# da-moon/noise-erasurecode-plugin

Hardware: AMD Instinct MI355X
Metric: RS(10,4) encode+reconstruct GB/s at 1/8 GPUs; % HBM roofline (higher is better)
Workload: dtype u8

## Files before the change

noise-erasurecode-plugin_amd/csrc/host_pipeline.cpp:

```cpp
#include "host_pipeline.hpp"

#include <algorithm>
#include <atomic>
#include <chrono>
#include <cstdlib>
#include <cstdio>
#include <cstring>
#include <mutex>
#include <new>
#include <string>
#include <utility>
#include <vector>
#if defined(__x86_64__)
#include <emmintrin.h>
#endif

namespace rsmi {

namespace {
constexpr size_t kPart = size_t(1) << 20;
constexpr size_t kPartMin = size_t(1) << 20;
constexpr size_t kChunkBytes = size_t(8) << 20;
size_t round_up(size_t x, size_t a) { return (x + a - 1) / a * a; }

int pool_threads() {
    const char* e = std::getenv("RSMI_COPY_THREADS");
    int t = e ? std::atoi(e) : static_cast<int>(std::thread::hardware_concurrency());
    return std::max(1, std::min(t, 8));
}
}

namespace {
inline void cpu_relax() {
#if defined(__x86_64__) || defined(__i386__)
    __builtin_ia32_pause();
#elif defined(__aarch64__)
    asm volatile("yield");
#endif
}
}

namespace {
bool stage_nt() {
    static const bool on = [] {
        const char* e = std::getenv("RSMI_STAGE_NT");
        return !(e && std::atoi(e) == 0);
    }();
    return on;
}
}

void stage_copy(void* dst, const void* src, size_t n) {
#if defined(__x86_64__)
    if (stage_nt() && n >= 4096) {
        uint8_t* d = static_cast<uint8_t*>(dst);
        const uint8_t* s = static_cast<const uint8_t*>(src);
        const size_t head = (16u - (reinterpret_cast<uintptr_t>(d) & 15u)) & 15u;
        std::memcpy(d, s, head);
        d += head;
        s += head;
        n -= head;
        size_t i = 0;
        for (; i + 64 <= n; i += 64) {
            const __m128i a = _mm_loadu_si128(reinterpret_cast<const __m128i*>(s + i));
            const __m128i b = _mm_loadu_si128(reinterpret_cast<const __m128i*>(s + i + 16));
            const __m128i c = _mm_loadu_si128(reinterpret_cast<const __m128i*>(s + i + 32));
            const __m128i e = _mm_loadu_si128(reinterpret_cast<const __m128i*>(s + i + 48));
            _mm_stream_si128(reinterpret_cast<__m128i*>(d + i), a);
            _mm_stream_si128(reinterpret_cast<__m128i*>(d + i + 16), b);
            _mm_stream_si128(reinterpret_cast<__m128i*>(d + i + 32), c);
            _mm_stream_si128(reinterpret_cast<__m128i*>(d + i + 48), e);
        }
        for (; i + 16 <= n; i += 16)
            _mm_stream_si128(reinterpret_cast<__m128i*>(d + i), _mm_loadu_si128(reinterpret_cast<const __m128i*>(s + i)));
        std::memcpy(d + i, s + i, n - i);
        return;
    }
#endif
    std::memcpy(dst, src, n);
}

namespace {
bool trace_on() {
    static const bool on = [] {
        const char* e = std::getenv("RSMI_TRACE");
        return e && std::atoi(e) != 0;
    }();
    return on;
}
struct TraceCall {
    std::chrono::steady_clock::time_point t[24];
    const char* name[24];
    int n = 0;
};
thread_local TraceCall g_call;
struct TraceTotals {
    std::mutex mu;
    std::vector<std::pair<std::string, std::vector<double>>> phases;
    long calls = 0;
    ~TraceTotals() {
        if (!calls) return;
        std::fprintf(stderr, "RSMI_TRACE %ld calls, median / mean us per phase:\n", calls);
        double total = 0;
        for (auto& p : phases) {
            std::vector<double>& v = p.second;
            double sum = 0;
            for (double x : v) sum += x;
            std::sort(v.begin(), v.end());
            total += v[v.size() / 2];
            std::fprintf(stderr, "  %-28s %8.2f %8.2f  (%zu)\n", p.first.c_str(), v[v.size() / 2], sum / v.size(),
                         v.size());
        }
        std::fprintf(stderr, "  %-28s %8.2f (sum of medians)\n", "total", total);
    }
};
TraceTotals g_totals;
}

void trace_begin() {
    if (!trace_on()) return;
    g_call.n = 0;
    trace_mark("begin");
}

void trace_mark(const char* phase) {
    if (!trace_on() || g_call.n >= 24) return;
    g_call.t[g_call.n] = std::chrono::steady_clock::now();
    g_call.name[g_call.n++] = phase;
}

void trace_end() {
    if (!trace_on() || g_call.n == 0) return;
    trace_mark("end");
    std::lock_guard<std::mutex> lk(g_totals.mu);
    ++g_totals.calls;
    for (int i = 1; i < g_call.n; ++i) {
        const double us = std::chrono::duration<double, std::micro>(g_call.t[i] - g_call.t[i - 1]).count();
        auto it = std::find_if(g_totals.phases.begin(), g_totals.phases.end(),
                               [&](const auto& p) { return p.first == g_call.name[i]; });
        if (it == g_totals.phases.end()) {
            g_totals.phases.push_back({g_call.name[i], {}});
            it = g_totals.phases.end() - 1;
        }
        it->second.push_back(us);
    }
    g_call.n = 0;
}

void stage_fence() {
#if defined(__x86_64__)
    if (stage_nt()) _mm_sfence();
#endif
}

hipError_t wait_event(hipEvent_t ev) {
    static const int spin_us = [] {
        const char* e = std::getenv("RSMI_SYNC_SPIN_US");
        return e ? std::max(0, std::min(std::atoi(e), 100000)) : 200;
    }();
    static const int max_spinners = [] {
        const char* e = std::getenv("RSMI_SYNC_SPINNERS");
        return e ? std::max(0, std::atoi(e)) : 2;
    }();
    static const bool adaptive = [] {
        const char* e = std::getenv("RSMI_SYNC_ADAPTIVE");
        return !(e && std::atoi(e) == 0);
    }();
    static std::atomic<int> spinners{0};
    thread_local bool last_short = true;
    const auto t0 = std::chrono::steady_clock::now();
    if (spin_us > 0 && (last_short || !adaptive)) {
        if (spinners.fetch_add(1, std::memory_order_relaxed) < max_spinners) {
            const auto until = t0 + std::chrono::microseconds(spin_us);
            do {
                const hipError_t q = hipEventQuery(ev);
                if (q != hipErrorNotReady) {
                    spinners.fetch_sub(1, std::memory_order_relaxed);
                    return q;
                }
                cpu_relax();
            } while (std::chrono::steady_clock::now() < until);
        }
        spinners.fetch_sub(1, std::memory_order_relaxed);
    }
    const hipError_t r = hipEventSynchronize(ev);
    last_short = std::chrono::steady_clock::now() - t0 <= std::chrono::microseconds(spin_us);
    return r;
}

namespace {
void copy_pieces(const CopyPool::Piece* b, const CopyPool::Piece* e);
}

struct CopyPool::Async {
    Job job;
    bool queued = false;
};

void CopyPool::split(const std::vector<Piece>& pieces, size_t group_bytes, Job& job) const {
    size_t group = 0;
    job.bounds.push_back(0);
    for (const Piece& p : pieces)
        for (size_t o = 0; o < p.len; o += kPart) {
            const size_t len = std::min(kPart, p.len - o);
            job.pieces.push_back({static_cast<uint8_t*>(p.dst) + o, static_cast<const uint8_t*>(p.src) + o, len, p.nt});
            group += len;
            if (group >= group_bytes) {
                job.bounds.push_back(job.pieces.size());
                group = 0;
// ... 294 lines not shown
```

noise-erasurecode-plugin_amd/csrc/rsmi.cpp:

```cpp
#include "../../include/rsmi.h"

#include <hip/hip_runtime.h>

#include <sched.h>

#include <algorithm>
#include <functional>
#include <atomic>
#include <chrono>
#include <cmath>
#include <cstdio>
#include <thread>
#include <condition_variable>
#include <cstdlib>
#include <cstring>
#include <deque>
#include <map>
#include <memory>
#include <mutex>
#include <new>
#include <shared_mutex>
#include <string>
#include <vector>

// ... 80 lines not shown
    void* p = nullptr;
    size_t cap = 0;
    bool reserve_keep(size_t bytes, size_t used, hipStream_t s) {
        if (bytes <= cap) return true;
        const size_t want = std::max({bytes, size_t(4096), 4 * cap});
        void* np = nullptr;
        if (hipMallocAsync(&np, want, s) != hipSuccess) return false;
        if (p && used &&
            hipMemcpyAsync(np, p, std::min(used, cap), hipMemcpyDeviceToDevice, s) != hipSuccess) {
            (void)hipFreeAsync(np, s);
            return false;
        }
        if (p) (void)hipFreeAsync(p, s);
        p = np;
        cap = want;
        return true;
    }
    bool needs(size_t bytes) const { return bytes > cap; }
    void release() {
        if (p) {
            (void)hipFreeAsync(p, nullptr);
            (void)hipStreamSynchronize(nullptr);
        }
        p = nullptr;
        cap = 0;
    }
};

struct Staging {
    void* p = nullptr;
    void* dev = nullptr;
    size_t cap = 0;
    unsigned flags = hipHostMallocDefault;
    hipEvent_t done = nullptr;
    bool pending = false;
    std::vector<void*> retired;
    bool acquire(size_t bytes) {
        if (pending) {
            (void)hipEventSynchronize(done);
            pending = false;
        }
        if (!done && hipEventCreateWithFlags(&done, hipEventDisableTiming) != hipSuccess) return false;
        if (bytes <= cap) return true;
        const size_t want = std::max({bytes, size_t(1) << 16, 2 * cap});
        void* np = nullptr;
        if (hipHostMalloc(&np, want, flags) != hipSuccess) return false;
        if (p) retired.push_back(p);
        p = np;
        if (hipHostGetDevicePointer(&dev, np, 0) != hipSuccess) dev = np;
        cap = want;
        return true;
    }
    void release_after(hipStream_t s) {
        if (hipEventRecord(done, s) == hipSuccess) pending = true;
    }
    void destroy() {
        if (pending) (void)hipEventSynchronize(done);
        for (void* r : retired) (void)hipHostFree(r);
        retired.clear();
        if (p) (void)hipHostFree(p);
        if (done) (void)hipEventDestroy(done);
        p = nullptr;
        dev = nullptr;
        done = nullptr;
    }
};

}

constexpr size_t kBatchChunks = 4;
constexpr size_t kBatchChunksMax = 8;
constexpr size_t kBatchChunkMin = size_t(16) << 20;

using rsmi::PatKey;

namespace {

struct Lease {
    hipStream_t stream = nullptr;
    hipStream_t stream2 = nullptr;
    hipEvent_t dev_done = nullptr;
    std::atomic<bool> dev_pending{false};
    hipEvent_t ev[kBatchChunksMax] = {};
    Staging st_stripe;
    Staging st_batch, st_pieces;
    Staging st_onepat;
    Staging st_out;
    Staging st_in;
    Staging st_scrub;
    rsmi::MailboxHost* mb = nullptr;
    rsmi::MailboxHost* mb_dev = nullptr;
    rsmi::MailboxDev* mbd = nullptr;
    uint64_t mb_timeout = 0;
    DevBuf d_stripe_pat, d_batch, d_pack, d_pieces, d_onepat, d_scrub;
    std::unique_ptr<rsmi::HostPipeline> pipe;
    std::vector<uint32_t> pid, start;
    std::vector<uint64_t> sort_a, sort_b;
    std::vector<PatKey> miss_keys;
    size_t seen_uploaded = 0;
    uint64_t seen_tables = ~uint64_t(0);

    bool init() {
        static const bool wc = [] {
            const char* e = std::getenv("RSMI_STAGE_WC");
            return e && std::atoi(e) != 0;
        }();
        if (wc) st_in.flags = hipHostMallocWriteCombined;
        if (hipStreamCreateWithFlags(&stream, hipStreamNonBlocking) != hipSuccess) return false;
        if (hipEventCreateWithFlags(&dev_done, hipEventDisableTiming) != hipSuccess) return false;
        for (hipEvent_t& e : ev)
            if (hipEventCreateWithFlags(&e, hipEventDisableTiming) != hipSuccess) return false;
        return true;
    }
    void begin(hipStream_t s) {
        if (dev_pending.load()) (void)hipStreamWaitEvent(s, dev_done, 0);
    }
    void end(hipStream_t s) {
        if (hipEventRecord(dev_done, s) == hipSuccess) dev_pending.store(true);
    }
    rsmi::HostPipeline* pipeline() {
        if (!pipe) pipe.reset(new (std::nothrow) rsmi::HostPipeline());
        return pipe.get();
    }
    hipStream_t chunk_stream(int ch) {
        static const bool two = [] {
            const char* e = std::getenv("RSMI_CHUNK_STREAMS");
            return e && std::atoi(e) == 2;
        }();
        if (!two || ch % 2 == 0) return stream;
        if (!stream2 && hipStreamCreateWithFlags(&stream2, hipStreamNonBlocking) != hipSuccess) stream2 = nullptr;
        return stream2 ? stream2 : stream;
    }
    ~Lease() {
        if (stream2) (void)hipStreamSynchronize(stream2);
        if (stream) (void)hipStreamSynchronize(stream);
        if (dev_pending.load()) (void)hipEventSynchronize(dev_done);
        pipe.reset();
        st_stripe.destroy();
        st_batch.destroy();
        st_pieces.destroy();
        st_onepat.destroy();
        st_out.destroy();
        st_in.destroy();
        st_scrub.destroy();
        for (DevBuf* b : {&d_stripe_pat, &d_batch, &d_pack, &d_pieces, &d_onepat, &d_scrub}) b->release();
        if (mb) (void)hipHostFree(mb);
        if (mbd) (void)hipFree(mbd);
        for (hipEvent_t e : ev)
            if (e) (void)hipEventDestroy(e);
        if (dev_done) (void)hipEventDestroy(dev_done);
        if (stream2) (void)hipStreamDestroy(stream2);
        if (stream) (void)hipStreamDestroy(stream);
    }
};

}

struct rs_ctx {
    int k = 0, n = 0, m = 0, device = 0;
    std::vector<uint8_t> enc;
    rsmi::DeviceSet* set = nullptr;
    bool set_member = false;
    const rsmi::BitsliceKernel* bitslice = nullptr;
    bool bitslice_rec = false;
    int bitslice_rec_min_e = 1;
    uint32_t xcd = 1;
    uint32_t xcd_split_enc = 0;
    uint32_t xcd_split_rec = ~0u;
    std::string rec_name;
    bool inline_desc = true;
    size_t small_split = 16;

    DevBuf d_encpat;
    DevBuf d_gf;

    mutable std::shared_mutex pat_mu;
    rsmi::PatIndex pat_index;
    std::vector<uint32_t> h_cnt;
    std::vector<uint8_t> h_lo;
    std::vector<rsmi::BsStripeMask> h_mask;
    int n_tops = 0;
    std::vector<PatKey> h_key;
    GrowBuf d_pcoef, d_psrc, d_pdst, d_pcnt, d_pstat, d_pkey;
    size_t uploaded = 0;
    size_t pat_cap = 0;
    int test_fail_flush = 0, flush_attempts = 0;
    uint64_t evictions = 0;
    uint64_t tables_gen = 0;
    std::atomic<int64_t> batches_in_place{0}, batches_staged{0};
    std::atomic<int64_t> encodes_in_place{0};
    std::atomic<int64_t> decodes_in_place{0};
    std::atomic<int64_t> rec_stripes_table{0}, rec_stripes_syndrome{0};
    std::atomic<int64_t> encode_batches{0};
    std::atomic<int64_t> mailbox_calls{0}, mailbox_recovered{0};
    std::atomic<int64_t> update_stripes{0}, update_copy_commits{0};
    std::atomic<int64_t> read_regenerated{0}, read_copied{0};
    std::atomic<int64_t> check_stripes{0}, scrub_regenerated{0};
    std::atomic<int64_t> repair_checked{0};
    std::atomic<int64_t> combine_jobs{0}, combine_rows{0};
    std::atomic<int64_t> batch_lens_passes{0};
    std::atomic<int64_t> combine_lens_launches{0};
    std::atomic<int64_t> update_degraded{0}, update_absorbed{0};
    std::atomic<int64_t> column_stripes{0}, column_bytes{0};
    bool repair_fused = true;
    uint32_t xcd_repair = 0;
    uint32_t xcd_update = ~0u;
    hipEvent_t pat_ev = nullptr;
    hipStream_t build_stream = nullptr;
    hipEvent_t caller_ev = nullptr;
    bool build_after_caller = true;
    bool pat_ev_valid = false;
    Staging st_pat;

    std::mutex lease_mu;
    std::condition_variable lease_cv;
    std::vector<std::unique_ptr<Lease>> leases;
    std::deque<Lease*> free_leases;
    size_t max_leases = 16;
};


namespace {

int hip_status(hipError_t e) { return e == hipSuccess ? RS_OK : RS_EDEVICE; }

Lease* acquire_lease(rs_ctx* c) {
    std::unique_lock<std::mutex> lk(c->lease_mu);
    c->lease_cv.wait(lk, [&] { return !c->free_leases.empty() || c->leases.size() < c->max_leases; });
    if (!c->free_leases.empty()) {
        Lease* L = c->free_leases.front();
        c->free_leases.pop_front();
        return L;
// ... 2856 lines not shown
        ptrs[i] = shares[order[i]];
    }
    std::copy(nums.begin(), nums.end(), numbers);
    std::copy(ptrs.begin(), ptrs.end(), shares);
    std::vector<uint8_t> present(n, 0);
    std::vector<const uint8_t*> by_id(n, nullptr);
    int distinct = 0;
    for (int i = 0; i < count; ++i)
        if (!present[nums[i]]) {
            present[nums[i]] = 1;
            by_id[nums[i]] = ptrs[i];
            ++distinct;
        }
    if (distinct < k) return RS_ESINGULAR;
    if (share_len == 0) return RS_OK;
    for (int i = 0; i < n; ++i)
        if (present[i] && !by_id[i]) return RS_EINVAL;
    if (c->set) {
        const SetPick pk(c->set);
        return rs_decode(pk.member(), numbers, shares, count, share_len, dst);
    }
    std::vector<uint8_t> aside;
    {
        OutRanges out;
        out.add(dst, static_cast<size_t>(k) * share_len);
        out.seal();
        set_aside_aliases(out, by_id, share_len, aside);
    }
    DeviceGuard g(c->device);
    if (!g.ok) return RS_EDEVICE;
    LeaseGuard lg(c);
    if (!lg.L) return RS_ENOMEM;
    rsmi::trace_mark("validate+lease");
    if (distinct > k) return correct_decode(c, *lg.L, present, by_id, share_len, dst);
    int rc_in_place = RS_OK;
    if (decode_in_place(c, *lg.L, present, by_id, share_len, dst, &rc_in_place)) return rc_in_place;
    return rebuild_into(c, *lg.L, present, by_id, share_len, dst);
}

namespace {
size_t batch_stage_cap() {
    static const size_t cap = [] {
        const char* e = std::getenv("RSMI_BATCH_STAGE_MB");
        const long v = e ? std::atol(e) : 0;
        return (v > 0 ? static_cast<size_t>(v) : size_t(512)) << 20;
    }();
    return cap;
}

int sort_message(int k, int n, int cnt, int* nb, const uint8_t** sb, std::vector<const uint8_t*>& by_id) {
    if (cnt < k) return RS_ENOT_ENOUGH;
    for (int i = 0; i < cnt; ++i)
        if (nb[i] < 0 || nb[i] >= n) return RS_EBAD_SHARE_ID;
    std::vector<int> order(cnt);
    for (int i = 0; i < cnt; ++i) order[i] = i;
    std::stable_sort(order.begin(), order.end(), [&](int x, int y) { return nb[x] < nb[y]; });
    std::vector<int> nums(cnt);
    std::vector<const uint8_t*> ptrs(cnt);
    for (int i = 0; i < cnt; ++i) {
        nums[i] = nb[order[i]];
        ptrs[i] = sb[order[i]];
    }
    std::copy(nums.begin(), nums.end(), nb);
    std::copy(ptrs.begin(), ptrs.end(), sb);
    by_id.assign(n, nullptr);
    int distinct = 0;
    for (int i = 0; i < cnt; ++i)
        if (!by_id[nums[i]]) {
            by_id[nums[i]] = ptrs[i];
            ++distinct;
        }
    return distinct < k ? RS_ESINGULAR : distinct > k ? 1 : static_cast<int>(RS_OK);
}

size_t direct_batch_chunks(size_t messages, size_t in_bytes) {
    static const size_t cap = [] {
        const char* e = std::getenv("RSMI_BATCH_CHUNKS");
        const long v = e ? std::atol(e) : static_cast<long>(kBatchChunks);
        return static_cast<size_t>(std::max(1L, std::min(v, static_cast<long>(kBatchChunksMax))));
    }();
    const size_t by_bytes = std::max<size_t>(1, in_bytes / (size_t(256) << 10));
    return std::max<size_t>(1, std::min({messages, cap, by_bytes}));
}
}

int rs_decode_batch(rs_ctx* c, int batch, const int* counts, int* numbers, const uint8_t** shares,
                    size_t S, uint8_t** dsts, int* status) {
    if (!c || batch < 0 || (batch && (!counts || !numbers || !shares || !dsts || !status)))
        return RS_EINVAL;
    rsmi::trace_begin();
    struct TraceEnd {
        ~TraceEnd() { rsmi::trace_end(); }
    } trace_end_at_exit;
    if (c->set) return rsmi::set_decode_batch(c->set, batch, counts, numbers, shares, S, dsts, status);
    const int k = c->k, n = c->n;
    if (batch > 0 && S > 0) {
        size_t total = 0;
        for (int b = 0; b < batch; ++b) total += static_cast<size_t>(std::max(counts[b], 0));
        OutRanges out;
        for (int b = 0; b < batch; ++b) out.add(dsts[b], static_cast<size_t>(k) * S);
        out.seal();
        std::vector<const uint8_t*> loc(shares, shares + total), orig(loc);
        std::vector<uint8_t> aside;
        if (set_aside_aliases(out, loc, S, aside)) {
            const int rc = rs_decode_batch(c, batch, counts, numbers, loc.data(), S, dsts, status);
            const uintptr_t a0 = reinterpret_cast<uintptr_t>(aside.data()), a1 = a0 + aside.size();
            std::vector<const uint8_t*> moved;
            for (const uint8_t* p : orig)
                if (p && out.meets(p, S)) moved.push_back(p);
            for (size_t j = 0; j < total; ++j) {
                const uintptr_t v = reinterpret_cast<uintptr_t>(loc[j]);
                shares[j] = (v >= a0 && v < a1) ? moved[(v - a0) / S] : loc[j];
            }
            return rc;
        }
    }
    {
        const size_t per_msg = 2 * static_cast<size_t>(k) * round_up(std::max<size_t>(S, 1), 256);
        const size_t group = std::max<size_t>(1, batch_stage_cap() / per_msg);
        if (static_cast<size_t>(batch) > group) {
            int rc = RS_OK;
            size_t off = 0;
            for (int b0 = 0; b0 < batch;) {
                const int nb = static_cast<int>(std::min<size_t>(group, static_cast<size_t>(batch - b0)));
                size_t cnt = 0;
                for (int b = b0; b < b0 + nb; ++b) cnt += static_cast<size_t>(std::max(counts[b], 0));
                const int r = rs_decode_batch(c, nb, counts + b0, numbers + off, shares + off, S, dsts + b0, status + b0);
                if (r != RS_OK && rc == RS_OK) rc = r;
                off += cnt;
                b0 += nb;
            }
            return rc;
        }
    }
    std::vector<size_t> first(batch + 1, 0);
    for (int b = 0; b < batch; ++b) first[b + 1] = first[b] + static_cast<size_t>(std::max(counts[b], 0));
    std::vector<int> fast;
    std::vector<std::vector<const uint8_t*>> by(batch);
    for (int b = 0; b < batch; ++b) {
        status[b] = sort_message(k, n, counts[b], numbers + first[b], shares + first[b], by[b]);
        if (status[b] == RS_OK && S > 0) fast.push_back(b);
    }
    for (int b = 0; b < batch; ++b) {
        if (status[b] != 1) continue;
        status[b] = rs_decode(c, numbers + first[b], shares + first[b], counts[b], S, dsts[b]);
    }
    auto first_fail = [&] {
        for (int b = 0; b < batch; ++b)
            if (status[b] != RS_OK) return status[b];
        return static_cast<int>(RS_OK);
    };
    if (fast.empty()) return first_fail();
    if (fast.size() == 1) {
        const int b = fast[0];
        status[b] = rs_decode(c, numbers + first[b], shares + first[b], counts[b], S, dsts[b]);
        return first_fail();
    }
    auto fast_path = [&]() -> int {
        const size_t pitch = round_up(S, 256);
        const size_t B = fast.size();
        std::vector<uint8_t> erased(B * static_cast<size_t>(n), 0);
        std::vector<rsmi::CopyPool::Piece> in, direct;
        std::vector<uint8_t*> regen;
        size_t n_par_out = 0;
        for (size_t j = 0; j < B; ++j)
            for (int i = 0; i < n; ++i) {
                const uint8_t* p = by[fast[j]][i];
                if (p) {
                    if (i < k) direct.push_back({dsts[fast[j]] + static_cast<size_t>(i) * S, p, S});
                } else {
                    erased[j * n + i] = 1;
                    if (i < k) regen.push_back(dsts[fast[j]] + static_cast<size_t>(i) * S);
                    else ++n_par_out;
                }
            }
        const size_t E = regen.size();
        const size_t out_rows = E + n_par_out;
        const size_t sb = round_up(S, 16);
        std::vector<uint64_t> dev_of(B * static_cast<size_t>(n), 0);
        bool in_place = std::getenv("RSMI_NO_DIRECT") == nullptr;
        for (size_t j = 0; j < B && in_place; ++j)
            for (int i = 0; i < n && in_place; ++i)
                if (const uint8_t* p = by[fast[j]][i]) {
                    const uint64_t d = (reinterpret_cast<uintptr_t>(p) & 15u) ? 0 : rsmi::pinned_device_address(p, sb);
                    in_place = d != 0;
                    dev_of[j * n + i] = d;
                }
        const size_t packed = in_place ? 0 : B * static_cast<size_t>(k) * pitch;
        ++(in_place ? c->batches_in_place : c->batches_staged);
        DeviceGuard g(c->device);
        if (!g.ok) return RS_EDEVICE;
        LeaseGuard lg(c);
        if (!lg.L) return RS_ENOMEM;
        Lease& L = *lg.L;
        rsmi::HostPipeline* pipe = L.pipeline();
        if (!pipe) return RS_ENOMEM;
        const hipStream_t s = L.stream;
        static const bool batch_dma = [] {
            const char* e = std::getenv("RSMI_BATCH_DMA");
            return e && std::atoi(e) != 0;
        }();
        if (!batch_dma) {
            const size_t sp = round_up(S, 64);
            const size_t in_bytes = in_place ? 0 : B * static_cast<size_t>(k) * sp;
            const size_t tbl = B * static_cast<size_t>(n) * sizeof(uint64_t);
            L.begin(s);
            struct StagingDone {
                Lease& L;
                hipStream_t s;
                ~StagingDone() {
                    L.st_batch.release_after(s);
                    L.end(s);
                }
            } staging_done{L, s};
            if (!L.st_batch.acquire(in_bytes + std::max<size_t>(E, 1) * sp) || !L.st_pieces.acquire(tbl) ||
                !L.d_pieces.reserve_on(tbl, s) || !L.d_batch.reserve_on(std::max<size_t>(n_par_out, 1) * sp, s))
                return RS_ENOMEM;
            uint8_t* h = static_cast<uint8_t*>(L.st_batch.p);
            uint8_t* hd = static_cast<uint8_t*>(L.st_batch.dev);
            uint8_t* h_out = h + in_bytes;
            uint8_t* d_out = hd + in_bytes;
            uint8_t* d_par = static_cast<uint8_t*>(L.d_batch.p);
            uint64_t* tab = static_cast<uint64_t*>(L.st_pieces.p);
            std::vector<rsmi::CopyPool::Piece> stage_in;
            stage_in.reserve(B * static_cast<size_t>(k));
            size_t r_data = 0, r_par = 0;
            for (size_t j = 0; j < B; ++j) {
                size_t q = 0;
                for (int i = 0; i < n; ++i) {
                    uint64_t& t = tab[j * n + i];
                    if (const uint8_t* p = by[fast[j]][i]) {
                        const size_t slot = j * k + q++;
                        if (in_place) {
                            t = dev_of[j * n + i];
                        } else {
                            stage_in.push_back({h + slot * sp, p, S, true});
                            t = reinterpret_cast<uint64_t>(hd + slot * sp);
                        }
                    } else if (i < k) {
                        t = reinterpret_cast<uint64_t>(d_out + r_data++ * sp);
                    } else {
                        t = reinterpret_cast<uint64_t>(d_par + r_par++ * sp);
                    }
                }
            }
            auto finish = [&](int code) {
                if (hipStreamSynchronize(s) != hipSuccess && code == RS_OK) code = RS_EDEVICE;
                return code;
            };
            if (hipMemcpyAsync(L.d_pieces.p, tab, tbl, hipMemcpyHostToDevice, s) != hipSuccess) return finish(RS_EDEVICE);
            L.st_pieces.release_after(s);
            const size_t moved = B * static_cast<size_t>(k) * sp;
            const size_t nch = direct_batch_chunks(B, moved);
            std::vector<size_t> rows_before(B + 1, 0);
            for (size_t j = 0; j < B; ++j) {
                size_t e_j = 0;
                for (int i = 0; i < k; ++i) e_j += by[fast[j]][i] == nullptr;
                rows_before[j + 1] = rows_before[j] + e_j;
            }
            size_t launched = 0;
            static const char* const kStage[] = {"stage0", "stage1", "stage2", "stage3", "stage4", "stage5", "stage6", "stage7"};
            static const char* const kLaunch[] = {"launch0", "launch1", "launch2", "launch3",
                                                  "launch4", "launch5", "launch6", "launch7"};
            static const char* const kWait[] = {"wait0", "wait1", "wait2", "wait3", "wait4", "wait5", "wait6", "wait7"};
            static const char* const kOut[] = {"copyout0", "copyout1", "copyout2", "copyout3",
                                               "copyout4", "copyout5", "copyout6", "copyout7"};
            static_assert(kBatchChunksMax == 8, "trace phase names");
            for (size_t ch = 0; ch < nch; ++ch) {
                const size_t j0 = B * ch / nch, j1 = B * (ch + 1) / nch;
                if (!in_place)
                    pipe->copy(std::vector<rsmi::CopyPool::Piece>(stage_in.begin() + j0 * k, stage_in.begin() + j1 * k));
                rsmi::trace_mark(kStage[ch]);
                const int st = reconstruct(c, L, StripeView::ptrs(sp, S), j1 - j0, erased.data() + j0 * n,
                                           static_cast<const uint64_t*>(L.d_pieces.p) + j0 * n, s);
                if (st != RS_OK || hipEventRecord(L.ev[ch], s) != hipSuccess) return finish(st != RS_OK ? st : RS_EDEVICE);
                rsmi::trace_mark(kLaunch[ch]);
                ++launched;
            }
            pipe->copy(direct);
            rsmi::trace_mark("copy_present");
            for (size_t ch = 0; ch < launched; ++ch) {
                if (rsmi::wait_event(L.ev[ch]) != hipSuccess) return finish(RS_EDEVICE);
                rsmi::trace_mark(kWait[ch]);
                const size_t j0 = B * ch / nch, j1 = B * (ch + 1) / nch;
                std::vector<rsmi::CopyPool::Piece> out;
                for (size_t r = rows_before[j0]; r < rows_before[j1]; ++r) out.push_back({regen[r], h_out + r * sp, S});
                pipe->copy(out);
                rsmi::trace_mark(kOut[ch]);
            }
            return RS_OK;
        }
        L.begin(s);
        const size_t table_bytes = B * static_cast<size_t>(n) * sizeof(uint64_t);
        if (!L.st_batch.acquire(std::max<size_t>(std::max(packed, E * pitch), 16)) ||
            (packed && !L.d_pack.reserve_on(packed, s)) || !L.d_batch.reserve_on(std::max<size_t>(out_rows, 1) * pitch, s) ||
            !L.st_pieces.acquire(table_bytes) || !L.d_pieces.reserve_on(table_bytes, s))
            return RS_ENOMEM;
        auto finish = [&](int code) {
            if (hipStreamSynchronize(s) != hipSuccess && code == RS_OK) code = RS_EDEVICE;
            L.end(s);
            return code;
        };
        uint8_t* h = static_cast<uint8_t*>(L.st_batch.p);
        uint8_t* dp = static_cast<uint8_t*>(L.d_pack.p);
        uint8_t* dout = static_cast<uint8_t*>(L.d_batch.p);
        uint64_t* tab = static_cast<uint64_t*>(L.st_pieces.p);
        size_t r_data = 0, r_par = E;
        for (size_t j = 0; j < B; ++j) {
            size_t q = 0;
            for (int i = 0; i < n; ++i) {
                uint64_t& t = tab[j * n + i];
                if (const uint8_t* p = by[fast[j]][i]) {
                    const size_t slot = j * k + q++;
                    if (in_place) {
                        t = dev_of[j * n + i];
                    } else {
                        in.push_back({h + slot * pitch, p, S});
                        t = reinterpret_cast<uint64_t>(dp + slot * pitch);
                    }
                } else {
                    t = reinterpret_cast<uint64_t>(dout + (i < k ? r_data++ : r_par++) * pitch);
                }
            }
        }
        if (hipMemcpyAsync(L.d_pieces.p, tab, table_bytes, hipMemcpyHostToDevice, s) != hipSuccess)
            return finish(RS_EDEVICE);
        L.st_pieces.release_after(s);
        const size_t chunks = in_place ? 0 : std::min<size_t>(B, packed >= kBatchChunkMin ? kBatchChunks : 1);
        for (size_t ch = 0; ch < chunks; ++ch) {
            const size_t j0 = B * ch / chunks, j1 = B * (ch + 1) / chunks;
            pipe->copy(std::vector<rsmi::CopyPool::Piece>(in.begin() + j0 * k, in.begin() + j1 * k));
            if (hipMemcpyAsync(dp + j0 * k * pitch, h + j0 * k * pitch, (j1 - j0) * k * pitch, hipMemcpyHostToDevice, s) !=
                hipSuccess)
                return finish(RS_EDEVICE);
        }
        const int st = reconstruct(c, L, StripeView::ptrs(pitch, S), B, erased.data(),
                                   static_cast<const uint64_t*>(L.d_pieces.p), s);
        if (st != RS_OK) return finish(st);
        const size_t ochunks = E == 0 ? 0 : std::min<size_t>(E, E * pitch >= kBatchChunkMin ? kBatchChunks : 1);
        int rc_dev = RS_OK;
        size_t queued = 0;
        for (size_t ch = 0; ch < ochunks && rc_dev == RS_OK; ++ch, ++queued) {
            const size_t r0 = E * ch / ochunks, r1 = E * (ch + 1) / ochunks;
            if (hipMemcpyAsync(h + r0 * pitch, dout + r0 * pitch, (r1 - r0) * pitch, hipMemcpyDeviceToHost, s) !=
                    hipSuccess ||
                hipEventRecord(L.ev[ch], s) != hipSuccess)
                rc_dev = RS_EDEVICE;
        }
        if (rc_dev == RS_OK) pipe->copy(direct);
        for (size_t ch = 0; ch < queued && rc_dev == RS_OK; ++ch) {
            const size_t r0 = E * ch / ochunks, r1 = E * (ch + 1) / ochunks;
            if (hipEventSynchronize(L.ev[ch]) != hipSuccess) {
                rc_dev = RS_EDEVICE;
                break;
            }
            std::vector<rsmi::CopyPool::Piece> out;
            out.reserve(r1 - r0);
            for (size_t r = r0; r < r1; ++r) out.push_back({regen[r], h + r * pitch, S});
            pipe->copy(out);
        }
        const int fin = finish(rc_dev);
        L.st_batch.release_after(s);
        return fin;
    };
    const int fr = fast_path();
    if (fr != RS_OK)
        for (int b : fast) status[b] = fr;
    return first_fail();
}

int rs_encode_batch(rs_ctx* c, int batch, const uint8_t* const* inputs, size_t len, uint8_t* const* parities,
                    int* status) {
    if (!c || batch < 0 || (batch && (!inputs || !parities || !status))) return RS_EINVAL;
    rsmi::trace_begin();
    struct TraceEnd {
        ~TraceEnd() { rsmi::trace_end(); }
    } trace_end_at_exit;
    if (c->set) return rsmi::set_encode_batch(c->set, batch, inputs, len, parities, status);
    const size_t k = static_cast<size_t>(c->k), m = static_cast<size_t>(c->m);
    if (len % k != 0) {
        for (int b = 0; b < batch; ++b) status[b] = RS_ELEN_NOT_MULTIPLE;
        return batch ? RS_ELEN_NOT_MULTIPLE : RS_OK;
    }
    const size_t S = len / k;
    int rc = RS_OK;
    std::vector<int> todo;
    for (int b = 0; b < batch; ++b) {
        status[b] = RS_OK;
        if (S == 0 || m == 0) continue;
        if (!inputs[b] || !parities[b]) {
            status[b] = RS_EINVAL;
            if (rc == RS_OK) rc = RS_EINVAL;
            continue;
        }
        todo.push_back(b);
    }
    if (todo.empty()) return rc;
    const size_t pitch = round_up(S, 64);
    const size_t per_msg = (k + m) * pitch;
    if (todo.size() == 1 || per_msg > batch_stage_cap() || round_up(S, 16) / 16 >= (size_t(1) << 28)) {
        for (int b : todo) status[b] = rs_encode(c, inputs[b], len, parities[b]);
        for (int b = 0; b < batch; ++b)
            if (status[b] != RS_OK) return status[b];
        return RS_OK;
    }
    auto fail_from = [&](size_t j0, int code) {
        for (size_t j = j0; j < todo.size(); ++j) status[todo[j]] = code;
        for (int b = 0; b < batch; ++b)
            if (status[b] != RS_OK) return status[b];
        return code;
    };
    DeviceGuard g(c->device);
    if (!g.ok) return fail_from(0, RS_EDEVICE);
    LeaseGuard lg(c);
    if (!lg.L) return fail_from(0, RS_ENOMEM);
    Lease& L = *lg.L;
    rsmi::HostPipeline* pipe = L.pipeline();
    if (!pipe) return fail_from(0, RS_ENOMEM);
    const hipStream_t s = L.stream;
    const size_t group = std::max<size_t>(1, batch_stage_cap() / per_msg);
    for (size_t g0 = 0; g0 < todo.size(); g0 += group) {
        const size_t B = std::min(group, todo.size() - g0);
        if (!L.st_batch.acquire(B * per_msg)) return fail_from(g0, RS_ENOMEM);
        uint8_t* h_in = static_cast<uint8_t*>(L.st_batch.p);
        uint8_t* h_out = h_in + B * k * pitch;
        uint8_t* d_in = static_cast<uint8_t*>(L.st_batch.dev);
        uint8_t* d_out = d_in + B * k * pitch;
        L.begin(s);
        const size_t nch = direct_batch_chunks(B, B * k * pitch);
        hipError_t e = hipSuccess;
        size_t launched = 0;
        for (size_t ch = 0; ch < nch && e == hipSuccess; ++ch) {
            const size_t j0 = B * ch / nch, j1 = B * (ch + 1) / nch;
            std::vector<rsmi::CopyPool::Piece> in;
            in.reserve((j1 - j0) * k);
            for (size_t j = j0; j < j1; ++j)
                for (size_t i = 0; i < k; ++i)
                    in.push_back({h_in + (j * k + i) * pitch, inputs[todo[g0 + j]] + i * S, S, true});
            pipe->copy(in);
            rsmi::trace_mark(ch == 0 ? "stage0" : ch == 1 ? "stage1" : ch == 2 ? "stage2" : "stage3");
            rsmi::MatArgs a = base_args(c, StripeView{d_in + j0 * k * pitch, k * pitch, d_out + j0 * m * pitch, m * pitch, pitch, S},
                                        j1 - j0);
            set_patterns(c, 1, c->d_encpat.p, a);
            a.stripe_desc = nullptr;
            e = launch_encode(c, a, s);
            if (e == hipSuccess) e = hipEventRecord(L.ev[ch], s);
            if (e == hipSuccess) ++launched;
            rsmi::trace_mark(ch == 0 ? "launch0" : ch == 1 ? "launch1" : ch == 2 ? "launch2" : "launch3");
        }
        L.end(s);
        for (size_t ch = 0; ch < launched && e == hipSuccess; ++ch) {
            e = rsmi::wait_event(L.ev[ch]);
            rsmi::trace_mark(ch == 0 ? "wait0" : ch == 1 ? "wait1" : ch == 2 ? "wait2" : "wait3");
            if (e != hipSuccess) break;
            const size_t j0 = B * ch / nch, j1 = B * (ch + 1) / nch;
            std::vector<rsmi::CopyPool::Piece> out;
            out.reserve((j1 - j0) * m);
            for (size_t j = j0; j < j1; ++j)
                for (size_t t = 0; t < m; ++t) out.push_back({parities[todo[g0 + j]] + t * S, h_out + (j * m + t) * pitch, S});
            pipe->copy(out);
            rsmi::trace_mark(ch == 0 ? "copyout0" : ch == 1 ? "copyout1" : ch == 2 ? "copyout2" : "copyout3");
        }
        if (e != hipSuccess) {
            (void)hipStreamSynchronize(s);
            for (size_t j = g0; j < todo.size(); ++j) status[todo[j]] = RS_EDEVICE;
            break;
        }
        c->encode_batches += 1;
    }
    (void)rc;
    for (int b = 0; b < batch; ++b)
        if (status[b] != RS_OK) return status[b];
    return RS_OK;
}

namespace {
struct LensMsg {
    size_t S = 0;
    std::vector<const uint8_t*> src;
    std::vector<uint64_t> src_dev;
    std::vector<uint8_t*> out;
    uint32_t coef = 0;
};

int lens_pass(rs_ctx* c, Lease& L, const std::vector<LensMsg>& msgs, const std::vector<uint8_t>& coef,
              const std::function<void()>& while_gpu) {
    const size_t B = msgs.size(), k = static_cast<size_t>(c->k);
    rsmi::HostPipeline* pipe = L.pipeline();
    if (!pipe) return RS_ENOMEM;
    const hipStream_t s = L.stream;
    size_t in_bytes = 0, out_bytes = 0, moved = 0;
    rsmi::CombinePlan plan;
    for (const LensMsg& m : msgs) {
        const size_t sp = round_up(m.S, 64);
        if (m.src_dev.empty()) in_bytes += k * sp;
        out_bytes += m.out.size() * sp;
        moved += k * sp;
        plan.max_nout = std::max<uint32_t>(plan.max_nout, static_cast<uint32_t>(m.out.size()));
        plan.rows += m.out.size();
    }
    if (!L.st_batch.acquire(in_bytes + out_bytes)) return RS_ENOMEM;
    uint8_t* h = static_cast<uint8_t*>(L.st_batch.p);
    const uint64_t hd = reinterpret_cast<uint64_t>(L.st_batch.dev);
    plan.max_nsrc = static_cast<uint32_t>(k);
    plan.mg = rsmi::combine_row_group(plan.max_nsrc, plan.max_nout);
    plan.groups = (plan.max_nout + plan.mg - 1) / plan.mg;
    plan.iters = rsmi::combine_iters_cap();
    plan.coef = coef;
    plan.live = static_cast<uint32_t>(B);
    std::vector<size_t> in_off(B), out_off(B);
    size_t in_at = 0, out_at = in_bytes;
    for (size_t j = 0; j < B; ++j) {
        const LensMsg& m = msgs[j];
        const size_t sp = round_up(m.S, 64);
        plan.jobs.push_back(rsmi::CombineJob{static_cast<uint32_t>(plan.addrs.size()), m.coef, static_cast<uint16_t>(k),
                                             static_cast<uint16_t>(m.out.size()), 0});
        in_off[j] = in_at;
        out_off[j] = out_at;
        for (size_t i = 0; i < k; ++i) plan.addrs.push_back(m.src_dev.empty() ? hd + in_at + i * sp : m.src_dev[i]);
        if (m.src_dev.empty()) in_at += k * sp;
        for (size_t t = 0; t < m.out.size(); ++t) plan.addrs.push_back(hd + out_at + t * sp);
        out_at += m.out.size() * sp;
        plan.ncols.push_back(static_cast<uint32_t>(round_up(m.S, 16) / 16));
    }
    const size_t nch = direct_batch_chunks(B, moved);
    std::vector<size_t> cut(nch + 1, B);
    cut[0] = 0;
    {
        size_t j = 0, bytes = 0;
        for (size_t ch = 0; ch + 1 < nch; ++ch) {
            const size_t want = moved / nch * (ch + 1);
            do bytes += k * round_up(msgs[j++].S, 64);
            while (bytes < want && j < B - (nch - 1 - ch));
            cut[ch + 1] = j;
        }
    }
    for (size_t ch = 0; ch < nch; ++ch) {
        uint64_t blocks = 0;
        for (size_t j = cut[ch]; j < cut[ch + 1]; ++j) {
            plan.first_block.push_back(static_cast<uint32_t>(blocks));
            blocks += static_cast<uint64_t>(rsmi::combine_lens_chunks(plan.ncols[j], plan.iters)) * plan.groups;
        }
        if (blocks > 0x7FFFFFFFull) return RS_EINVAL;
        plan.first_block.push_back(static_cast<uint32_t>(blocks));
    }
    rsmi::CombLensArgs a{};
    a.mg = plan.mg;
    a.groups = plan.groups;
    a.iters = plan.iters;
    const int up = upload_combine_lens(c, L, plan, s, &a);
    if (up != RS_OK) return up;
    const rsmi::CombLensArgs base = a;
    hipError_t e = hipSuccess;
    size_t launched = 0;
    for (size_t ch = 0; ch < nch && e == hipSuccess; ++ch) {
        const size_t j0 = cut[ch], j1 = cut[ch + 1];
        std::vector<rsmi::CopyPool::Piece> in;
        for (size_t j = j0; j < j1; ++j) {
            if (!msgs[j].src_dev.empty()) continue;
            const size_t sp = round_up(msgs[j].S, 64);
            for (size_t i = 0; i < k; ++i) in.push_back({h + in_off[j] + i * sp, msgs[j].src[i], msgs[j].S, true});
        }
        pipe->copy(in);
        a = base;
        a.jobs = base.jobs + j0;
        a.ncols = base.ncols + j0;
        a.first_block = base.first_block + j0 + ch;
        a.njobs = static_cast<uint32_t>(j1 - j0);
        e = rsmi::launch_combine_lens(a, plan.max_nsrc, plan.first_block[j1 + ch], s);
        if (e == hipSuccess) e = hipEventRecord(L.ev[ch], s);
        if (e == hipSuccess) ++launched;
    }
    L.end(s);
    if (e == hipSuccess && while_gpu) while_gpu();
    for (size_t ch = 0; ch < launched && e == hipSuccess; ++ch) {
        e = rsmi::wait_event(L.ev[ch]);
        if (e != hipSuccess) break;
        std::vector<rsmi::CopyPool::Piece> out;
        for (size_t j = cut[ch]; j < cut[ch + 1]; ++j) {
            const size_t sp = round_up(msgs[j].S, 64);
            for (size_t t = 0; t < msgs[j].out.size(); ++t) out.push_back({msgs[j].out[t], h + out_off[j] + t * sp, msgs[j].S});
        }
        pipe->copy(out);
    }
    if (e != hipSuccess) {
        (void)hipStreamSynchronize(s);
        return RS_EDEVICE;
    }
    ++c->batch_lens_passes;
    return RS_OK;
}

void lens_groups(const std::vector<size_t>& need, const std::vector<uint8_t>& alone, std::vector<size_t>& ends) {
    for (size_t g0 = 0; g0 < need.size();) {
        size_t g1 = g0, bytes = 0;
        while (g1 < need.size()) {
            const bool single = alone[g1] || need[g1] > batch_stage_cap();
            if (g1 > g0 && (single || bytes + need[g1] > batch_stage_cap())) break;
            bytes += need[g1++];
            if (single) break;
        }
        ends.push_back(g1);
        g0 = g1;
    }
}
}

int rs_encode_batch_lens(rs_ctx* c, int batch, const uint8_t* const* inputs, const size_t* lens, uint8_t* const* parities,
                         int* status) {
    if (!c || batch < 0 || (batch && (!inputs || !lens || !parities || !status))) return RS_EINVAL;
    rsmi::trace_begin();
    struct TraceEnd {
        ~TraceEnd() { rsmi::trace_end(); }
    } trace_end_at_exit;
    if (c->set) return rsmi::set_encode_batch_lens(c->set, batch, inputs, lens, parities, status);
    const size_t k = static_cast<size_t>(c->k), m = static_cast<size_t>(c->m);
    std::vector<int> todo;
    for (int b = 0; b < batch; ++b) {
        status[b] = RS_OK;
        if (lens[b] % k != 0) status[b] = RS_ELEN_NOT_MULTIPLE;
        else if (lens[b] == 0 || m == 0) continue;
        else if (!inputs[b] || !parities[b]) status[b] = RS_EINVAL;
        else todo.push_back(b);
    }
    auto first_fail = [&] {
        for (int b = 0; b < batch; ++b)
            if (status[b] != RS_OK) return status[b];
        return static_cast<int>(RS_OK);
    };
    if (todo.empty()) return first_fail();
    bool one_len = true;
    for (int b : todo) one_len &= lens[b] == lens[todo[0]];
    if (one_len) {
        std::vector<const uint8_t*> in;
        std::vector<uint8_t*> par;
        for (int b : todo) in.push_back(inputs[b]), par.push_back(parities[b]);
        std::vector<int> st(todo.size(), RS_OK);
        (void)rs_encode_batch(c, static_cast<int>(todo.size()), in.data(), lens[todo[0]], par.data(), st.data());
        for (size_t j = 0; j < todo.size(); ++j) status[todo[j]] = st[j];
        return first_fail();
    }
    std::vector<size_t> need(todo.size());
    std::vector<uint8_t> alone(todo.size(), 0);
    for (size_t j = 0; j < todo.size(); ++j) {
        const size_t S = lens[todo[j]] / k;
        need[j] = (k + m) * round_up(S, 64);
        alone[j] = round_up(S, 16) / 16 >= (size_t(1) << 28);
    }
    const std::vector<uint8_t> bottom(c->enc.begin() + static_cast<ptrdiff_t>(k * k), c->enc.end());
    std::vector<size_t> ends;
    lens_groups(need, alone, ends);
    size_t g0 = 0;
    for (size_t g1 : ends) {
        if (g1 - g0 == 1) {
            const int b = todo[g0];
            status[b] = rs_encode(c, inputs[b], lens[b], parities[b]);
        } else {
            std::vector<LensMsg> msgs(g1 - g0);
            for (size_t j = g0; j < g1; ++j) {
                const int b = todo[j];
                LensMsg& msg = msgs[j - g0];
                msg.S = lens[b] / k;
                for (size_t i = 0; i < k; ++i) msg.src.push_back(inputs[b] + i * msg.S);
                for (size_t t = 0; t < m; ++t) msg.out.push_back(parities[b] + t * msg.S);
            }
            int rc = RS_OK;
            {
                DeviceGuard g(c->device);
                LeaseGuard lg(c);
// ... 401 lines not shown
```

Measured before the change: 6068.

## Stage batch inputs/outputs through device buffers via DMA copy streams

```diff
diff --git a/noise-erasurecode-plugin_amd/csrc/host_pipeline.cpp b/noise-erasurecode-plugin_amd/csrc/host_pipeline.cpp
--- a/noise-erasurecode-plugin_amd/csrc/host_pipeline.cpp
+++ b/noise-erasurecode-plugin_amd/csrc/host_pipeline.cpp
@@ -89,8 +89,8 @@
     return on;
 }
 struct TraceCall {
-    std::chrono::steady_clock::time_point t[24];
-    const char* name[24];
+    std::chrono::steady_clock::time_point t[40];
+    const char* name[40];
     int n = 0;
 };
 thread_local TraceCall g_call;
@@ -124,7 +124,7 @@
 }
 
 void trace_mark(const char* phase) {
-    if (!trace_on() || g_call.n >= 24) return;
+    if (!trace_on() || g_call.n >= 40) return;
     g_call.t[g_call.n] = std::chrono::steady_clock::now();
     g_call.name[g_call.n++] = phase;
 }
diff --git a/noise-erasurecode-plugin_amd/csrc/rsmi.cpp b/noise-erasurecode-plugin_amd/csrc/rsmi.cpp
--- a/noise-erasurecode-plugin_amd/csrc/rsmi.cpp
+++ b/noise-erasurecode-plugin_amd/csrc/rsmi.cpp
@@ -186,6 +186,9 @@
     hipEvent_t dev_done = nullptr;
     std::atomic<bool> dev_pending{false};
     hipEvent_t ev[kBatchChunksMax] = {};
+    hipStream_t stream_copy = nullptr;
+    hipEvent_t ev_x[kBatchChunksMax] = {}, ev_y[kBatchChunksMax] = {};
+    hipEvent_t ev_ready = nullptr;
     Staging st_stripe;
     Staging st_batch, st_pieces;
     Staging st_onepat;
@@ -197,6 +200,7 @@
     rsmi::MailboxDev* mbd = nullptr;
     uint64_t mb_timeout = 0;
     DevBuf d_stripe_pat, d_batch, d_pack, d_pieces, d_onepat, d_scrub;
+    DevBuf d_stage;
     std::unique_ptr<rsmi::HostPipeline> pipe;
     std::vector<uint32_t> pid, start;
     std::vector<uint64_t> sort_a, sort_b;
@@ -235,7 +239,17 @@
         if (!stream2 && hipStreamCreateWithFlags(&stream2, hipStreamNonBlocking) != hipSuccess) stream2 = nullptr;
         return stream2 ? stream2 : stream;
     }
+    bool copy_lane() {
+        if (stream_copy) return true;
+        for (hipEvent_t* set : {ev_x, ev_y})
+            for (size_t i = 0; i < kBatchChunksMax; ++i)
+                if (!set[i] && hipEventCreateWithFlags(&set[i], hipEventDisableTiming) != hipSuccess) return false;
+        if (!ev_ready && hipEventCreateWithFlags(&ev_ready, hipEventDisableTiming) != hipSuccess) return false;
+        if (hipStreamCreateWithFlags(&stream_copy, hipStreamNonBlocking) != hipSuccess) stream_copy = nullptr;
+        return stream_copy != nullptr;
+    }
     ~Lease() {
+        if (stream_copy) (void)hipStreamSynchronize(stream_copy);
         if (stream2) (void)hipStreamSynchronize(stream2);
         if (stream) (void)hipStreamSynchronize(stream);
         if (dev_pending.load()) (void)hipEventSynchronize(dev_done);
@@ -247,11 +261,17 @@
         st_out.destroy();
         st_in.destroy();
         st_scrub.destroy();
-        for (DevBuf* b : {&d_stripe_pat, &d_batch, &d_pack, &d_pieces, &d_onepat, &d_scrub}) b->release();
+        for (DevBuf* b : {&d_stripe_pat, &d_batch, &d_pack, &d_pieces, &d_onepat, &d_scrub, &d_stage}) b->release();
         if (mb) (void)hipHostFree(mb);
         if (mbd) (void)hipFree(mbd);
         for (hipEvent_t e : ev)
             if (e) (void)hipEventDestroy(e);
+        for (hipEvent_t e : ev_x)
+            if (e) (void)hipEventDestroy(e);
+        for (hipEvent_t e : ev_y)
+            if (e) (void)hipEventDestroy(e);
+        if (ev_ready) (void)hipEventDestroy(ev_ready);
+        if (stream_copy) (void)hipStreamDestroy(stream_copy);
         if (dev_done) (void)hipEventDestroy(dev_done);
         if (stream2) (void)hipStreamDestroy(stream2);
         if (stream) (void)hipStreamDestroy(stream);
@@ -3274,6 +3294,82 @@
     const size_t by_bytes = std::max<size_t>(1, in_bytes / (size_t(256) << 10));
     return std::max<size_t>(1, std::min({messages, cap, by_bytes}));
 }
+
+enum class BatchForm { kDirect, kH2D, kD2H, kDma, kBoth };
+enum class BatchCall { kEncode, kDecode, kLens };
+BatchForm batch_form(BatchCall call) {
+    static const int forced = [] {
+        if (const char* e = std::getenv("RSMI_BATCH_FORM")) {
+            static const char* const kNames[] = {"direct", "h2d", "d2h", "dma", "both"};
+            for (int i = 0; i < 5; ++i)
+                if (std::strcmp(e, kNames[i]) == 0) return i;
+        }
+        const char* d = std::getenv("RSMI_BATCH_DMA");
+        return d && std::atoi(d) != 0 ? static_cast<int>(BatchForm::kDma) : -1;
+    }();
+    if (forced >= 0) return static_cast<BatchForm>(forced);
+    static constexpr BatchForm kDefault[] = {BatchForm::kBoth, BatchForm::kBoth, BatchForm::kDirect};
+    return kDefault[static_cast<int>(call)];
+}
+
+struct CopyLane {
+    Lease& L;
+    const hipStream_t s;
+    const BatchForm form;
+    uint8_t* dev_in = nullptr;
+    uint8_t* dev_out = nullptr;
+    hipStream_t s_out = nullptr;
+    bool used = false;
+    CopyLane(Lease& l, hipStream_t st, BatchForm f) : L(l), s(st), form(f) {}
+    bool h2d() const { return form == BatchForm::kH2D || form == BatchForm::kBoth; }
+    bool d2h() const { return form == BatchForm::kD2H || form == BatchForm::kBoth; }
+    bool open(size_t in_bytes, size_t out_bytes) {
+        if (!h2d() && !d2h()) return true;
+        const size_t in_room = h2d() ? round_up(in_bytes, 256) : 0;
+        if (!L.copy_lane() || !L.d_stage.reserve_on(std::max<size_t>(in_room + (d2h() ? out_bytes : 0), 16), s)) return false;
+        dev_in = static_cast<uint8_t*>(L.d_stage.p);
+        dev_out = dev_in + in_room;
+        s_out = L.stream_copy;
+        if (form == BatchForm::kBoth) {
+            if (!L.stream2 && hipStreamCreateWithFlags(&L.stream2, hipStreamNonBlocking) != hipSuccess) L.stream2 = nullptr;
+            if (!L.stream2) return false;
+            s_out = L.stream2;
+        }
+        if (hipEventRecord(L.ev_ready, s) != hipSuccess || hipStreamWaitEvent(L.stream_copy, L.ev_ready, 0) != hipSuccess)
+            return false;
+        used = true;
+        return true;
+    }
+    hipError_t in(size_t ch, size_t off, const uint8_t* host, size_t bytes) {
+        if (!h2d() || bytes == 0) return hipSuccess;
+        hipError_t e = hipMemcpyAsync(dev_in + off, host, bytes, hipMemcpyHostToDevice, L.stream_copy);
+        if (e == hipSuccess) e = hipEventRecord(L.ev_x[ch], L.stream_copy);
+        if (e == hipSuccess) e = hipStreamWaitEvent(s, L.ev_x[ch], 0);
+        return e;
+    }
+    hipError_t out(size_t ch, size_t off, uint8_t* host, size_t bytes) {
+        if (!d2h()) return hipEventRecord(L.ev[ch], s);
+        hipError_t e = hipEventRecord(L.ev_y[ch], s);
+        if (e == hipSuccess) e = hipStreamWaitEvent(s_out, L.ev_y[ch], 0);
+        if (e == hipSuccess && bytes) e = hipMemcpyAsync(host, dev_out + off, bytes, hipMemcpyDeviceToHost, s_out);
+        if (e == hipSuccess) e = hipEventRecord(L.ev[ch], s_out);
+        return e;
+    }
+    void join(size_t launched) {
+        if (d2h() && launched) (void)hipStreamWaitEvent(s, L.ev[launched - 1], 0);
+    }
+    void drain() {
+        if (!used) return;
+        (void)hipStreamSynchronize(L.stream_copy);
+        if (s_out != L.stream_copy) (void)hipStreamSynchronize(s_out);
+    }
+};
+
+const char* const kStage[] = {"stage0", "stage1", "stage2", "stage3", "stage4", "stage5", "stage6", "stage7"};
+const char* const kLaunch[] = {"launch0", "launch1", "launch2", "launch3", "launch4", "launch5", "launch6", "launch7"};
+const char* const kWait[] = {"wait0", "wait1", "wait2", "wait3", "wait4", "wait5", "wait6", "wait7"};
+const char* const kOut[] = {"copyout0", "copyout1", "copyout2", "copyout3", "copyout4", "copyout5", "copyout6", "copyout7"};
+static_assert(kBatchChunksMax == 8, "trace phase names");
 }
 
 int rs_decode_batch(rs_ctx* c, int batch, const int* counts, int* numbers, const uint8_t** shares,
@@ -3388,11 +3484,8 @@
         rsmi::HostPipeline* pipe = L.pipeline();
         if (!pipe) return RS_ENOMEM;
         const hipStream_t s = L.stream;
-        static const bool batch_dma = [] {
-            const char* e = std::getenv("RSMI_BATCH_DMA");
-            return e && std::atoi(e) != 0;
-        }();
-        if (!batch_dma) {
+        const BatchForm form = batch_form(BatchCall::kDecode);
+        if (form != BatchForm::kDma) {
             const size_t sp = round_up(S, 64);
             const size_t in_bytes = in_place ? 0 : B * static_cast<size_t>(k) * sp;
             const size_t tbl = B * static_cast<size_t>(n) * sizeof(uint64_t);
@@ -3408,10 +3501,13 @@
             if (!L.st_batch.acquire(in_bytes + std::max<size_t>(E, 1) * sp) || !L.st_pieces.acquire(tbl) ||
                 !L.d_pieces.reserve_on(tbl, s) || !L.d_batch.reserve_on(std::max<size_t>(n_par_out, 1) * sp, s))
                 return RS_ENOMEM;
+            CopyLane lane(L, s, in_place ? BatchForm::kDirect : form);
+            if (!lane.open(in_bytes, E * sp)) return RS_ENOMEM;
             uint8_t* h = static_cast<uint8_t*>(L.st_batch.p);
             uint8_t* hd = static_cast<uint8_t*>(L.st_batch.dev);
+            uint8_t* d_in = lane.h2d() ? lane.dev_in : hd;
             uint8_t* h_out = h + in_bytes;
-            uint8_t* d_out = hd + in_bytes;
+            uint8_t* d_out = lane.d2h() ? lane.dev_out : hd + in_bytes;
             uint8_t* d_par = static_cast<uint8_t*>(L.d_batch.p);
             uint64_t* tab = static_cast<uint64_t*>(L.st_pieces.p);
             std::vector<rsmi::CopyPool::Piece> stage_in;
@@ -3427,7 +3523,7 @@
                             t = dev_of[j * n + i];
                         } else {
                             stage_in.push_back({h + slot * sp, p, S, true});
-                            t = reinterpret_cast<uint64_t>(hd + slot * sp);
+                            t = reinterpret_cast<uint64_t>(d_in + slot * sp);
                         }
                     } else if (i < k) {
                         t = reinterpret_cast<uint64_t>(d_out + r_data++ * sp);
@@ -3438,6 +3534,7 @@
             }
             auto finish = [&](int code) {
                 if (hipStreamSynchronize(s) != hipSuccess && code == RS_OK) code = RS_EDEVICE;
+                lane.drain();
                 return code;
             };
             if (hipMemcpyAsync(L.d_pieces.p, tab, tbl, hipMemcpyHostToDevice, s) != hipSuccess) return finish(RS_EDEVICE);
@@ -3451,24 +3548,21 @@
                 rows_before[j + 1] = rows_before[j] + e_j;
             }
             size_t launched = 0;
-            static const char* const kStage[] = {"stage0", "stage1", "stage2", "stage3", "stage4", "stage5", "stage6", "stage7"};
-            static const char* const kLaunch[] = {"launch0", "launch1", "launch2", "launch3",
-                                                  "launch4", "launch5", "launch6", "launch7"};
-            static const char* const kWait[] = {"wait0", "wait1", "wait2", "wait3", "wait4", "wait5", "wait6", "wait7"};
-            static const char* const kOut[] = {"copyout0", "copyout1", "copyout2", "copyout3",
-                                               "copyout4", "copyout5", "copyout6", "copyout7"};
-            static_assert(kBatchChunksMax == 8, "trace phase names");
             for (size_t ch = 0; ch < nch; ++ch) {
                 const size_t j0 = B * ch / nch, j1 = B * (ch + 1) / nch;
                 if (!in_place)
                     pipe->copy(std::vector<rsmi::CopyPool::Piece>(stage_in.begin() + j0 * k, stage_in.begin() + j1 * k));
+                if (lane.in(ch, j0 * k * sp, h + j0 * k * sp, (j1 - j0) * k * sp) != hipSuccess) return finish(RS_EDEVICE);
                 rsmi::trace_mark(kStage[ch]);
                 const int st = reconstruct(c, L, StripeView::ptrs(sp, S), j1 - j0, erased.data() + j0 * n,
                                            static_cast<const uint64_t*>(L.d_pieces.p) + j0 * n, s);
-                if (st != RS_OK || hipEventRecord(L.ev[ch], s) != hipSuccess) return finish(st != RS_OK ? st : RS_EDEVICE);
+                if (st != RS_OK || lane.out(ch, rows_before[j0] * sp, h_out + rows_before[j0] * sp,
+                                            (rows_before[j1] - rows_before[j0]) * sp) != hipSuccess)
+                    return finish(st != RS_OK ? st : RS_EDEVICE);
                 rsmi::trace_mark(kLaunch[ch]);
                 ++launched;
             }
+            lane.join(launched);
             pipe->copy(direct);
             rsmi::trace_mark("copy_present");
             for (size_t ch = 0; ch < launched; ++ch) {
@@ -3619,6 +3713,13 @@
         uint8_t* d_in = static_cast<uint8_t*>(L.st_batch.dev);
         uint8_t* d_out = d_in + B * k * pitch;
         L.begin(s);
+        CopyLane lane(L, s, batch_form(BatchCall::kEncode));
+        if (!lane.open(B * k * pitch, B * m * pitch)) {
+            L.end(s);
+            return fail_from(g0, RS_ENOMEM);
+        }
+        if (lane.h2d()) d_in = lane.dev_in;
+        if (lane.d2h()) d_out = lane.dev_out;
         const size_t nch = direct_batch_chunks(B, B * k * pitch);
         hipError_t e = hipSuccess;
         size_t launched = 0;
@@ -3630,20 +3731,23 @@
                 for (size_t i = 0; i < k; ++i)
                     in.push_back({h_in + (j * k + i) * pitch, inputs[todo[g0 + j]] + i * S, S, true});
             pipe->copy(in);
-            rsmi::trace_mark(ch == 0 ? "stage0" : ch == 1 ? "stage1" : ch == 2 ? "stage2" : "stage3");
+            e = lane.in(ch, j0 * k * pitch, h_in + j0 * k * pitch, (j1 - j0) * k * pitch);
+            rsmi::trace_mark(kStage[ch]);
+            if (e != hipSuccess) break;
             rsmi::MatArgs a = base_args(c, StripeView{d_in + j0 * k * pitch, k * pitch, d_out + j0 * m * pitch, m * pitch, pitch, S},
                                         j1 - j0);
             set_patterns(c, 1, c->d_encpat.p, a);
             a.stripe_desc = nullptr;
             e = launch_encode(c, a, s);
-            if (e == hipSuccess) e = hipEventRecord(L.ev[ch], s);
+            if (e == hipSuccess) e = lane.out(ch, j0 * m * pitch, h_out + j0 * m * pitch, (j1 - j0) * m * pitch);
             if (e == hipSuccess) ++launched;
-            rsmi::trace_mark(ch == 0 ? "launch0" : ch == 1 ? "launch1" : ch == 2 ? "launch2" : "launch3");
-        }
+            rsmi::trace_mark(kLaunch[ch]);
+        }
+        lane.join(launched);
         L.end(s);
         for (size_t ch = 0; ch < launched && e == hipSuccess; ++ch) {
             e = rsmi::wait_event(L.ev[ch]);
-            rsmi::trace_mark(ch == 0 ? "wait0" : ch == 1 ? "wait1" : ch == 2 ? "wait2" : "wait3");
+            rsmi::trace_mark(kWait[ch]);
             if (e != hipSuccess) break;
             const size_t j0 = B * ch / nch, j1 = B * (ch + 1) / nch;
             std::vector<rsmi::CopyPool::Piece> out;
@@ -3651,10 +3755,11 @@
             for (size_t j = j0; j < j1; ++j)
                 for (size_t t = 0; t < m; ++t) out.push_back({parities[todo[g0 + j]] + t * S, h_out + (j * m + t) * pitch, S});
             pipe->copy(out);
-            rsmi::trace_mark(ch == 0 ? "copyout0" : ch == 1 ? "copyout1" : ch == 2 ? "copyout2" : "copyout3");
+            rsmi::trace_mark(kOut[ch]);
         }
         if (e != hipSuccess) {
             (void)hipStreamSynchronize(s);
+            lane.drain();
             for (size_t j = g0; j < todo.size(); ++j) status[todo[j]] = RS_EDEVICE;
             break;
         }
@@ -3694,6 +3799,23 @@
     if (!L.st_batch.acquire(in_bytes + out_bytes)) return RS_ENOMEM;
     uint8_t* h = static_cast<uint8_t*>(L.st_batch.p);
     const uint64_t hd = reinterpret_cast<uint64_t>(L.st_batch.dev);
+    BatchForm form = batch_form(BatchCall::kLens);
+    for (const LensMsg& m : msgs)
+        if (!m.src_dev.empty()) {
+            if (form == BatchForm::kD2H) form = BatchForm::kDirect;
+            if (form == BatchForm::kBoth) form = BatchForm::kH2D;
+        }
+    if (form == BatchForm::kH2D && in_bytes == 0) form = BatchForm::kDirect;
+    CopyLane lane(L, s, form);
+    if (lane.h2d() || lane.d2h()) {
+        L.begin(s);
+        if (!lane.open(in_bytes, out_bytes)) {
+            L.end(s);
+            return RS_ENOMEM;
+        }
+    }
+    const uint64_t in_dev = lane.h2d() ? reinterpret_cast<uint64_t>(lane.dev_in) : hd;
+    const uint64_t out_dev = lane.d2h() ? reinterpret_cast<uint64_t>(lane.dev_out) : hd + in_bytes;
     plan.max_nsrc = static_cast<uint32_t>(k);
     plan.mg = rsmi::combine_row_group(plan.max_nsrc, plan.max_nout);
     plan.groups = (plan.max_nout + plan.mg - 1) / plan.mg;
@@ -3709,9 +3831,9 @@
                                              static_cast<uint16_t>(m.out.size()), 0});
         in_off[j] = in_at;
         out_off[j] = out_at;
-        for (size_t i = 0; i < k; ++i) plan.addrs.push_back(m.src_dev.empty() ? hd + in_at + i * sp : m.src_dev[i]);
+        for (size_t i = 0; i < k; ++i) plan.addrs.push_back(m.src_dev.empty() ? in_dev + in_at + i * sp : m.src_dev[i]);
         if (m.src_dev.empty()) in_at += k * sp;
-        for (size_t t = 0; t < m.out.size(); ++t) plan.addrs.push_back(hd + out_at + t * sp);
+        for (size_t t = 0; t < m.out.size(); ++t) plan.addrs.push_back(out_dev + (out_at - in_bytes) + t * sp);
         out_at += m.out.size() * sp;
         plan.ncols.push_back(static_cast<uint32_t>(round_up(m.S, 16) / 16));
     }
@@ -3754,15 +3876,19 @@
             for (size_t i = 0; i < k; ++i) in.push_back({h + in_off[j] + i * sp, msgs[j].src[i], msgs[j].S, true});
         }
         pipe->copy(in);
+        const size_t in_end = j1 < B ? in_off[j1] : in_bytes, out_end = j1 < B ? out_off[j1] : in_bytes + out_bytes;
+        e = lane.in(ch, in_off[j0], h + in_off[j0], in_end - in_off[j0]);
+        if (e != hipSuccess) break;
         a = base;
         a.jobs = base.jobs + j0;
         a.ncols = base.ncols + j0;
         a.first_block = base.first_block + j0 + ch;
         a.njobs = static_cast<uint32_t>(j1 - j0);
         e = rsmi::launch_combine_lens(a, plan.max_nsrc, plan.first_block[j1 + ch], s);
-        if (e == hipSuccess) e = hipEventRecord(L.ev[ch], s);
+        if (e == hipSuccess) e = lane.out(ch, out_off[j0] - in_bytes, h + out_off[j0], out_end - out_off[j0]);
         if (e == hipSuccess) ++launched;
     }
+    lane.join(launched);
     L.end(s);
     if (e == hipSuccess && while_gpu) while_gpu();
     for (size_t ch = 0; ch < launched && e == hipSuccess; ++ch) {
@@ -3777,6 +3903,7 @@
     }
     if (e != hipSuccess) {
         (void)hipStreamSynchronize(s);
+        lane.drain();
         return RS_EDEVICE;
     }
     ++c->batch_lens_passes;
```

Result: no change. 6068, median of 2 (+0.0%).
